# bitsauce/Carla-ppo

Measured on AMD Instinct MI355X. Metric: VAE+PPO train frames/sec on 160×80×3 synthetic obs at 1/2/4/8 MI355X, higher is better.
Workload: dtype bf16; 1 GPU; ConvVAE SGD step (fwd+ELBO+bwd+TF-Adam), batch=512 per GPU, 160x80x3 frames, z_dim=64, rgb target (BASELINE configs[1]; global batch 512); global_batch=512, parallelism=single, frames_resident_in_hbm=2048, frame_table=uint8 camera bytes, k/255 in registers, noise=N(0,1) drawn inside the reparameterisation kernel (Philox4x32-10), launch=eager launches: one C call per step (mi_vae_train_step), storage=bf16 activations/weights, fp32 accumulate, fp32 master weights+Adam

## Files before the change

### carla-ppo_amd/csrc/conv_ops.hip

```cpp
#include <stdlib.h>
#include "gemm_core.hpp"
#include "tallk_tile.hpp"
#include "mi_internal.hpp"
#include "mi355_carla.h"

using namespace mi;

namespace {

inline int esz_of(int dtype) { return dtype == MI_BF16 ? 2 : 4; }
inline bool dtype_ok(int dtype) { return dtype == MI_F32 || dtype == MI_BF16 || dtype == MI_BF16X3; }

template <typename T, typename TIn, int AMODE, int BMODE, int VA, int AALIGN>
int launch_gemm_bn(hipStream_t st, const GemmParams& p, int M_for_grid, int gz) {
    const int gx = (M_for_grid + GEMM_BM - 1) / GEMM_BM;
    if (gx <= 0) return MI_OK;
    if (p.N <= 32) {
        dim3 g(gx, 1, gz);
        MI_LAUNCH((gemm_kernel<T, TIn, AMODE, BMODE, VA, AALIGN, 32>), g, dim3(GEMM_NT), 0, st, p);
    } else if (p.N <= 64) {
        dim3 g(gx, 1, gz);
        MI_LAUNCH((gemm_kernel<T, TIn, AMODE, BMODE, VA, AALIGN, 64>), g, dim3(GEMM_NT), 0, st, p);
    } else {
        dim3 g(gx, (p.N + 127) / 128, gz);
// ... 141 lines not shown
    if (j == 0) { f.first[0] = 0; f.ovw = 0; }
    if (overwrite) f.ovw |= 1u << j;
    f.slabs[j] = slabs; f.out[j] = out; f.stride[j] = stride; f.n[j] = n; f.nslab[j] = nslab;
    f.kl[j] = sr_kl(n, nslab);
    f.vec[j] = ((((uintptr_t)slabs) | ((uintptr_t)out)) & 15) == 0 && stride % 4 == 0;
    const long long quads = (n + 3) / 4;
    f.first[j + 1] = f.first[j] + (int)((quads * f.kl[j] + 255) / 256);
}
struct PendingReduce { TapWgradParams q; int splits, ngroups, kind; const float* bpart; float* bout; int bnslab, bN; };
struct PendingFold { const float* tmp; float* out; const float* tmp_bias; float* dbias; int T, R, Q, NB; };
static thread_local PendingFold g_folds[16];
static thread_local int g_nfolds = 0;
__global__ __launch_bounds__(256) void fold_split_kernel(const PendingFold f) {
    const long long n = (long long)f.T * f.R * f.Q;
    const long long i = (long long)blockIdx.x * 256 + threadIdx.x;
    if (i < n) {
        const int q = (int)(i % f.Q); const long long tr = i / f.Q; const int r = (int)(tr % f.R); const long long t = tr / f.R;
        const float* s = f.tmp + ((t * 2 * f.R + 2 * r) * 2ll * f.Q + 2 * q);
        f.out[i] += (s[0] + s[1]) + (s[2ll * f.Q] + s[2ll * f.Q + 1]);
    } else if (f.dbias && i - n < f.NB) {
        const int b = (int)(i - n);
        f.dbias[b] += f.tmp_bias[2 * b] + f.tmp_bias[2 * b + 1];
    }
}
static int launch_fold(hipStream_t st, const PendingFold& f) {
    const long long n = (long long)f.T * f.R * f.Q + (f.dbias ? f.NB : 0);
    MI_LAUNCH(fold_split_kernel, dim3((unsigned)((n + 255) / 256)), dim3(256), 0, st, f);
    return mi_check_launch("fold_split_kernel");
}
static thread_local PendingReduce g_pending[16];
static thread_local int g_npending = 0, g_defer_reduces = 0, g_defer_pause = 0;
static unsigned reduce_ry(const PendingReduce& r) {
    unsigned ry = 1;
    while (((unsigned)(r.ngroups / 512 + 1) * ry < 512 || r.splits / (int)ry > 16) && (int)(ry * 2) <= r.splits / 4 && ry < (unsigned)knob(K_REDUCE_RY_CAP)) ry *= 2;
    return ry;
}
static unsigned reduce_blocks(const PendingReduce& r, unsigned ry) { const unsigned upb = 256 / ry, nunits = (unsigned)r.ngroups / 2; return (nunits + upb - 1) / upb; }
static void launch_tiled_reduce(hipStream_t st, const PendingReduce& r) {
    const unsigned ry = reduce_ry(r);
    const dim3 rg(reduce_blocks(r, ry), 1, 1);
    if (r.kind == 0) MI_LAUNCH((reduce_tiled_kernel<TC_CONV, 2, 4, 2>), rg, dim3(256), 0, st, r.q, r.splits, r.ngroups, (int)ry);
    else if (r.kind == 1) MI_LAUNCH((reduce_tiled_kernel<TC_GATHER, 2, 4, 2>), rg, dim3(256), 0, st, r.q, r.splits, r.ngroups, (int)ry);
    else MI_LAUNCH((reduce_tiled_kernel<TC_GATHER, 3, 2, 4>), rg, dim3(256), 0, st, r.q, r.splits, r.ngroups, (int)ry);
    if (r.bpart) mi_reduce_slabs(st, r.bpart, (long long)r.bN, r.bnslab, (long long)r.bN, r.bout);
}
extern "C" int mi_tapwgrad_defer(int on) {
    const int prev = g_defer_reduces;
    g_defer_reduces = on ? 1 : 0;
    g_npending = 0; g_nfolds = 0; g_defer_pause = 0;
    return prev;
}
extern "C" int mi_tapwgrad_defer_pause(int pause) { const int prev = g_defer_pause; g_defer_pause = pause ? 1 : 0; return prev; }
static thread_local int t_slab_bf16 = -1;
static inline int slab_bf16_now() { return t_slab_bf16 >= 0 ? t_slab_bf16 : knob(K_SLAB_BF16_DEFAULT); }
extern "C" int mi_tapwgrad_slab_bf16(int on) { const int prev = t_slab_bf16; t_slab_bf16 = on < 0 ? -1 : (on ? 1 : 0); return prev; }
static int tapwgrad_flush_reduces(void* stream);
extern "C" int mi_tapwgrad_flush(void* stream) {
    int rc = tapwgrad_flush_reduces(stream);
    const int nf = g_nfolds;
    g_nfolds = 0;
    for (int i = 0; i < nf && rc == MI_OK; ++i) rc = launch_fold((hipStream_t)stream, g_folds[i]);
    return rc;
}
static int tapwgrad_flush_reduces(void* stream) {
    const int n = g_npending;
    g_npending = 0;
    if (n == 0) return MI_OK;
    if (n == 1 || n > TW_MAX_FUSED) {
        for (int i = 0; i < n; ++i) launch_tiled_reduce((hipStream_t)stream, g_pending[i]);
        return mi_check_launch("reduce_tiled_kernel");
    }
    static thread_local FusedReduceParams f;
    f.n = n; f.first[0] = 0; f.bias.njobs = 0; f.bias.first[0] = 0; f.bias.ovw = 0;
    for (int i = 0; i < n; ++i) {
        const PendingReduce& r = g_pending[i];
        f.q[i] = r.q; f.splits[i] = r.splits; f.ngroups[i] = r.ngroups; f.kind[i] = r.kind; f.ry[i] = (int)reduce_ry(r);
        f.first[i + 1] = f.first[i] + (int)reduce_blocks(r, (unsigned)f.ry[i]);
        if (r.bpart && f.bias.njobs < SR_MAX) sr_add(f.bias, r.bpart, (long long)r.bN, r.bnslab, (long long)r.bN, r.bout);
    }
    for (int i = n; i < TW_MAX_FUSED; ++i) f.first[i + 1] = f.first[n];
    for (int i = f.bias.njobs; i < SR_MAX; ++i) f.bias.first[i + 1] = f.bias.first[f.bias.njobs];
    MI_LAUNCH(reduce_fused_kernel, dim3((unsigned)(f.first[n] + f.bias.first[f.bias.njobs])), dim3(256), 0, (hipStream_t)stream, f);
    return mi_check_launch("reduce_fused_kernel");
}

int try_tapwgrad(hipStream_t st, int dtype, int mode, const void* a, const void* d, int B, int IH, int IW, int C, int OH, int OW, int N,
                 int KH, int KW, float* out, void* scratch, long long scratch_bytes, float* dbias) {
    if (!knob(K_TAPWGRAD) || dtype != MI_BF16) return 0;
    if (KH != KW || KH < 3 || KH > 6) return 0;
    if ((((uintptr_t)a) & 15) || (((uintptr_t)d) & 15) || C % 8 != 0 || N % 8 != 0) return 0;
    TapWgradParams q = {};
    const int taps = (KH + 1) / 2;
    int KCB, NEB;
    if (mode == TC_CONV) {
        if (taps != 2 || (4 * C) % 128 != 0 || N % 64 != 0) return 0;
        q.GH = OH + 1; q.GW = OW + 1; q.HY = q.HX = 0; q.KC = 4 * C; q.NE = N; KCB = 128; NEB = 64;
    } else {
        q.HY = q.HX = taps - 1;
        q.GH = (OH + 1) / 2 + q.HY; q.GW = (OW + 1) / 2 + q.HX; q.KC = C; q.NE = 4 * N;
        if (taps == 2) { if (C % 128 != 0 || N % 64 != 0) return 0; KCB = 128; NEB = 64; }
        else { if (C % 64 != 0 || N != 32) return 0; KCB = 64; NEB = 128; }
    }
    if ((taps - 1) * q.GW + taps - 1 > TC_MAXHALO) return 0;
    const long long MP = (long long)B * q.GH * q.GW, a_bytes = (long long)B * IH * IW * C * 2, d_bytes = (long long)B * OH * OW * N * 2;
    if (MP >= (1ll << 30) || !fits_desc(a_bytes) || !fits_desc(d_bytes)) return 0;
    q.a = a; q.a_bytes = (uint32_t)a_bytes; q.d = d; q.d_bytes = (uint32_t)d_bytes;
    q.B = B; q.IH = IH; q.IW = IW; q.C = C; q.OH = OH; q.OW = OW; q.N = N; q.KH = KH; q.KW = KW; q.MP = (int)MP;
    q.nkb = q.KC / KCB;
    const int gy = q.nkb * (q.NE / NEB);
    const int ntb = NEB / 32;
    q.npairs = 0;
    for (int tap = 0; tap < taps * taps; ++tap)
        for (int nt = 0; nt < ntb; ++nt) {
            bool valid = true;
            if (mode == TC_GATHER && NEB == 4 * N) {
                const int ta = tap / taps, tb = tap % taps;
                valid = (nt >> 1) + 2 * (q.HY - ta) < KH && (nt & 1) + 2 * (q.HX - tb) < KW;
            }
            if (valid) {
                if (q.npairs >= 32) return 0;
                bool first = true;
                for (int k = 0; k < q.npairs; ++k) if (q.pair_nt[k] == nt) first = false;
                q.pair_tap[q.npairs] = (unsigned char)tap; q.pair_nt[q.npairs] = (unsigned char)nt; q.pair_first[q.npairs] = first ? 1 : 0; ++q.npairs;
            }
        }
    {
        unsigned char t2[32], n2[32], f2[32];
        int k = 0;
        for (int pass = 0; pass < 2; ++pass)
            for (int i = 0; i < q.npairs; ++i)
                if ((q.pair_first[i] != 0) == (pass == 0)) { t2[k] = q.pair_tap[i]; n2[k] = q.pair_nt[i]; f2[k] = q.pair_first[i]; ++k; }
        for (int i = 0; i < q.npairs; ++i) { q.pair_tap[i] = t2[i]; q.pair_nt[i] = n2[i]; q.pair_first[i] = f2[i]; }
    }
    q.dbias = dbias;
    int splits = knob(K_TAPWGRAD_BLOCKS) / gy; if (splits < 1) splits = 1;
    long long pps = (MP + splits - 1) / splits; pps = (pps + TW_BP - 1) / TW_BP * TW_BP;
    splits = (int)((MP + pps - 1) / pps);
    q.pos_per_split = (int)pps;
    q.div_g = make_fastdiv(q.GH); q.div_gw = make_fastdiv(q.GW); q.div_n = make_fastdiv(N);
    q.div_2c = make_fastdiv(2 * C); q.div_c = make_fastdiv(C);
    q.out = out;
    q.trace = g_trace; q.trace_cap = g_trace_cap; q.dbg_cheap_addr = (knob(K_WGRAD_DBG) >= 2 && knob(K_WGRAD_DBG) <= 5) ? knob(K_WGRAD_DBG) : 0;
    const int kt_tiles = taps == 2 ? 4 : 2;
    const long long slab_floats = (long long)gy * q.npairs * kt_tiles * 1024;
    q.slabs = nullptr; q.slab_stride = slab_floats; q.slab_bf16 = slab_bf16_now() ? 1 : 0;
    const bool split = knob(K_TAPWGRAD_SPLIT) && taps == 2 && q.npairs == 8;
    const long long slab_bytes = ((long long)splits * slab_floats * (q.slab_bf16 ? 2 : 4) + 255) / 256 * 256;
    q.bias_part = nullptr; q.bias_nh = split ? 2 : 1;
    const long long bias_bytes = dbias ? (long long)splits * q.bias_nh * q.NE * 4 : 0;
    if (scratch && splits > 1 && (((uintptr_t)scratch) & 15) == 0 && scratch_bytes >= slab_bytes + bias_bytes && slab_floats < (1ll << 29) && (!dbias || N <= 256)) {
        q.slabs = (float*)scratch;
        if (dbias) q.bias_part = (float*)((char*)scratch + slab_bytes);
    }
    q.gx = splits; q.gy = gy;
    dim3 g((unsigned)((splits + 7) / 8 * 8 * gy), 1, 1);
    const bool ldec = (knob(K_TW_LDEC) & 1) && !q.dbg_cheap_addr && !q.trace, ldec_cw = (knob(K_TW_LDEC) & 2) && !q.dbg_cheap_addr && !q.trace;
    const bool dbg = q.dbg_cheap_addr != 0;
    if (mode == TC_CONV) {
        if (split && dbg) MI_LAUNCH((tapwgrad_kernel<TC_CONV, 2, 4, 2, 2, true, false, true>), g, dim3(TW_NT), 0, st, q);
        else if (split && ldec) MI_LAUNCH((tapwgrad_kernel<TC_CONV, 2, 4, 2, 2, true, true>), g, dim3(TW_NT), 0, st, q);
        else if (split) MI_LAUNCH((tapwgrad_kernel<TC_CONV, 2, 4, 2, 2, true>), g, dim3(TW_NT), 0, st, q);
        else MI_LAUNCH((tapwgrad_kernel<TC_CONV, 2, 4, 2, 1>), g, dim3(TW_NT), 0, st, q);
    } else if (taps == 2) {
        if (split && dbg) MI_LAUNCH((tapwgrad_kernel<TC_GATHER, 2, 4, 2, 2, true, false, true>), g, dim3(TW_NT), 0, st, q);
        else if (split && ldec) MI_LAUNCH((tapwgrad_kernel<TC_GATHER, 2, 4, 2, 2, true, true>), g, dim3(TW_NT), 0, st, q);
        else if (split) MI_LAUNCH((tapwgrad_kernel<TC_GATHER, 2, 4, 2, 2, true>), g, dim3(TW_NT), 0, st, q);
        else MI_LAUNCH((tapwgrad_kernel<TC_GATHER, 2, 4, 2, 1>), g, dim3(TW_NT), 0, st, q);
    }
    else {
        if (q.npairs > 32) return 0;
        if (knob(K_TAPWGRAD_CW) && KH == 5 && C == 64 && q.NE == 128 && q.KC == 64 && q.slabs) {
            if (dbg) MI_LAUNCH((tapwgrad_cw_kernel<false, true>), g, dim3(TWC_NT), 0, st, q);
            else if (ldec_cw) MI_LAUNCH(tapwgrad_cw_kernel<true>, g, dim3(TWC_NT), 0, st, q); else MI_LAUNCH(tapwgrad_cw_kernel<false>, g, dim3(TWC_NT), 0, st, q);
        }
        else MI_LAUNCH((tapwgrad_kernel<TC_GATHER, 3, 2, 4, 4>), g, dim3(TW_NT), 0, st, q);
    }
    int rc = mi_check_launch("tapwgrad_kernel");
    if (rc == MI_OK && q.slabs) {
        PendingReduce r;
        r.q = q; r.splits = splits; r.ngroups = (int)(slab_floats / 4); r.kind = mode == TC_CONV ? 0 : (taps == 2 ? 1 : 2);
        r.bpart = q.bias_part; r.bout = dbias; r.bnslab = splits * q.bias_nh * (q.NE / N); r.bN = N;
        if (g_defer_reduces && !g_defer_pause && g_npending < 16) g_pending[g_npending++] = r;
        else { launch_tiled_reduce(st, r); rc = mi_check_launch("reduce_tiled_kernel"); }
    }
    return rc == MI_OK ? 1 : rc;
}

int try_tapwgrad_split(hipStream_t st, int mode, const void* a, const void* d, int B, int IH, int IW, int C, int OH, int OW, int N,
                       int KH, int KW, float* out, void* scratch, long long scratch_bytes, float* dbias) {
    const int on = knob(K_X3_TAPWGRAD);
    if (!on || !scratch || (((uintptr_t)scratch) & 255)) return 0;
    const long long nw = (long long)KH * KW * C * N;
    const long long tmp_bytes = ((4 * nw + 2 * N) * 4 + 255) / 256 * 256;
    if (scratch_bytes < tmp_bytes + (1 << 20)) return 0;
    const int taps = (KH + 1) / 2;
    if (KH != KW || taps != 2) return 0;
    if (mode == TC_CONV ? ((8 * C) % 128 != 0 || (2 * N) % 64 != 0) : ((2 * C) % 128 != 0 || (2 * N) % 64 != 0)) return 0;
    if (on != 2 && (mode != TC_CONV || (long long)C * N > 64 * 128)) return 0;
    float* tmp = (float*)scratch; float* tb = tmp + 4 * nw;
    if (hipMemsetAsync(tmp, 0, (size_t)((4 * nw + 2 * N) * 4), st) != hipSuccess) return mi_fail(MI_ERR_LAUNCH, "try_tapwgrad_split: memset failed");
    const int r = try_tapwgrad(st, MI_BF16, mode, a, d, B, IH, IW, 2 * C, OH, OW, 2 * N, KH, KW, tmp, (char*)scratch + tmp_bytes, scratch_bytes - tmp_bytes, dbias ? tb : nullptr);
    if (r <= 0) return r;
    PendingFold f = {tmp, out, tb, dbias, KH * KW, mode == TC_CONV ? C : N, mode == TC_CONV ? N : C, N};
    if (g_defer_reduces && !g_defer_pause && g_nfolds < 16) { g_folds[g_nfolds++] = f; return 1; }
    const int rc = launch_fold(st, f);
    return rc == MI_OK ? 1 : rc;
}

template <typename T, int TAPS, int CPR>
int launch_gather_narrow(hipStream_t st, const TapParams& q) {
    dim3 g((q.MP + GN_BMT - 1) / GN_BMT);
    if (q.N == 3 && sizeof(T) == 2 && q.labels && q.loss_kind == 0 && knob(K_NARROW_LEAN)) MI_LAUNCH((gather_narrow_kernel<T, TAPS, CPR, 3, true>), g, dim3(GN_NT), 0, st, q);
    else if (q.N == 3) MI_LAUNCH((gather_narrow_kernel<T, TAPS, CPR, 3>), g, dim3(GN_NT), 0, st, q);
    else if (q.N == 1) MI_LAUNCH((gather_narrow_kernel<T, TAPS, CPR, 1>), g, dim3(GN_NT), 0, st, q);
    else MI_LAUNCH((gather_narrow_kernel<T, TAPS, CPR, 0>), g, dim3(GN_NT), 0, st, q);
    return mi_check_launch("gather_narrow_kernel");
}

struct NarrowLoss {
    const float* labels; const int* idx; long long stride; int kind; float inv_b; void* dlogits; float* lpart; float* bpart; int cap; int nblocks;
// ... 790 lines not shown
```

### carla-ppo_amd/csrc/mi_internal.hpp

```cpp
#pragma once
#include <hip/hip_runtime.h>
#include <hip/hip_ext.h>
#include "tuning.hpp"

enum { MI_F32 = 0, MI_BF16 = 1, MI_BF16X3 = 2 };
enum { MI_OK = 0, MI_ERR_ARG = -1, MI_ERR_SHAPE = -2, MI_ERR_LAUNCH = -3, MI_ERR_STATE = -4 };

extern thread_local hipEvent_t mi_tl_stop_event;
#define MI_LAUNCH(kernel, grid, block, shmem, stream, ...) do { \
        if (mi_tl_stop_event) { const hipEvent_t ev__ = mi_tl_stop_event; mi_tl_stop_event = nullptr; \
            hipExtLaunchKernelGGL(kernel, grid, block, shmem, stream, nullptr, ev__, 0, __VA_ARGS__); } \
        else hipLaunchKernelGGL(kernel, grid, block, shmem, stream, __VA_ARGS__); } while (0)

const void* mi_rwconv_take_wfrag();
bool mi_enc12_eligible(int dtype, int B, int FH, int FW);
int mi_fail(int code, const char* msg);
int mi_check_launch(const char* what);

extern "C" int mi_tapwgrad_defer(int on);
extern "C" int mi_tapwgrad_flush(void* stream);
extern "C" int mi_tapwgrad_defer_pause(int pause);
extern "C" int mi_tapwgrad_slab_bf16(int on);

int mi_try_rwconv_gather(hipStream_t st, int dtype, const void* a, const void* w, int B, int IH, int IW, int C, int OH, int OW, int N,
                         int KH, int KW, void* out, const float* bias, const void* mask, int relu, const void* mask_bits, void* bits_out, const void* wfrag);
int mi_try_rwconv_conv(hipStream_t st, int dtype, const void* a, const void* w, int B, int IH, int IW, int C, int OH, int OW, int N,
                       int KH, int KW, int ldb, void* out, const float* bias, const void* mask, int relu, const void* wfrag);
void mi_get_trace(long long** buf, int* cap);

int mi_reduce_slabs(hipStream_t st, const float* slabs, long long stride, int nslab, long long n, float* out, int overwrite = 0);
extern "C" int mi_small_reduce_defer(int on);
extern "C" int mi_small_reduce_flush(void* stream);
extern "C" int mi_small_reduce_bind(void* stream);
extern "C" int mi_small_reduce_deferring(void);
```

### carla-ppo_amd/csrc/tapwgrad_tile.hpp

```cpp
#pragma once
#include <type_traits>
#include "tapconv_tile.hpp"
#include "wgrad_tile.hpp"

namespace mi {

constexpr int TW_BP = 128;
constexpr int TW_NT = 512;
constexpr int TW_MAXPAIR = 32;

struct TapWgradParams {
    const void* a; uint32_t a_bytes;
    const void* d; uint32_t d_bytes;
    int B, IH, IW, C;
    int OH, OW, N;
    int KH, KW;
    int GH, GW, HY, HX;
    int KC, NE, MP;
    int nkb;
    int gx, gy;
    int pos_per_split;
    int npairs;
    unsigned char pair_tap[TW_MAXPAIR], pair_nt[TW_MAXPAIR], pair_first[TW_MAXPAIR];
    float* dbias;
    FastDiv div_g, div_gw, div_n, div_2c, div_c;
    float* out;
    float* slabs; long long slab_stride;
    float* bias_part; int bias_nh;
    int slab_bf16;
    long long* trace; int trace_cap;
    int dbg_cheap_addr;
};

#ifdef MI355_TW_SLAB_PLAIN
#define TW_SLAB_STORE(v, ptr) (*(ptr) = (v))
#else
#define TW_SLAB_STORE(v, ptr) __builtin_nontemporal_store((v), (ptr))
#endif
typedef uint32_t u32x4 __attribute__((ext_vector_type(4)));
typedef uint32_t tw_u32x2 __attribute__((ext_vector_type(2)));
__device__ __forceinline__ u32x4 make_srd(const void* base, uint32_t bytes) {
    const unsigned long long b = (unsigned long long)base;
    u32x4 r;
    r[0] = (uint32_t)b; r[1] = (uint32_t)(b >> 32) & 0xffffu; r[2] = bytes; r[3] = 0x00020000u;
    r[0] = __builtin_amdgcn_readfirstlane(r[0]); r[1] = __builtin_amdgcn_readfirstlane(r[1]);
    r[2] = __builtin_amdgcn_readfirstlane(r[2]); r[3] = __builtin_amdgcn_readfirstlane(r[3]);
    return r;
}
__device__ __forceinline__ void dma16_asm(const u32x4 srd, uint32_t lds_addr, uint32_t voff) {
    asm volatile("s_mov_b32 m0, %0\n\ts_nop 0\n\tbuffer_load_dwordx4 %1, %2, 0 offen lds"
                 :: "s"(lds_addr), "v"(voff), "s"(srd) : "memory", "m0");
}

template <int CPR> __device__ __forceinline__ int tw_swz(int row) {
    return CPR == 16 ? (row & 3) << 2 : ((row >> 1) & 1) << 2;
}

template <int MODE, int TAPS>
__device__ __forceinline__ bool tw_dw_index(const TapWgradParams& p, int kc0, int ne0, int tap, int kt, int nt, int row, int lcol, long long& base, long long& stride) {
    const int ta = tap / TAPS, tb = tap % TAPS;
    if constexpr (MODE == TC_CONV) {
        const int kc = kc0 + kt * 32 + row, ne = ne0 + nt * 32 + lcol;
        uint32_t phh, rem, pww, c;
        p.div_2c.divmod((uint32_t)(kc < p.KC ? kc : 0), phh, rem);
        p.div_c.divmod(rem, pww, c);
        const int kh = 2 * ta + (int)phh, kw = 2 * tb + (int)pww;
        base = ((long long)(kh * p.KW + kw) * p.C + c) * p.N + ne; stride = p.N;
        return kc < p.KC && ne < p.NE && kh < p.KH && kw < p.KW;
    } else {
        const int ne = ne0 + nt * 32 + row, kc = kc0 + kt * 32 + lcol;
        uint32_t cls, n;
        p.div_n.divmod((uint32_t)(ne < p.NE ? ne : 0), cls, n);
        const int kh = (int)(cls >> 1) + 2 * (p.HY - ta), kw = (int)(cls & 1) + 2 * (p.HX - tb);
        base = ((long long)(kh * p.KW + kw) * p.N + n) * p.C + kc; stride = p.C;
        return kc < p.KC && ne < p.NE && kh < p.KH && kw < p.KW;
    }
}

template <int MODE, int TAPS, int KT, int NTB, int PPW, bool SPLIT = false, bool LDEC = false, bool DBG = false>
__global__ __launch_bounds__(TW_NT) void tapwgrad_kernel(const TapWgradParams p) {
    const int dbgm = DBG ? p.dbg_cheap_addr : 0;
    static_assert(!SPLIT || (TAPS == 2 && NTB == 2 && PPW == NTB), "split layout: 4 taps x 2 position halves = 8 waves");
    typedef bf16_t T;
    constexpr int ESZ = 2, VE = 8;
    constexpr int KCB = 32 * KT, NEB = 32 * NTB;
    constexpr int PA = KCB * ESZ, PD = NEB * ESZ;
    constexpr int CPA = PA / 16, CPD = PD / 16;
    constexpr int SPI_A = 1024 / PA, SPI_D = 1024 / PD;
    constexpr int MAXSLOT = TW_BP + TC_MAXHALO;
    constexpr int NIA = (MAXSLOT / SPI_A + 7) / 8;
    constexpr int NID = TW_BP / SPI_D / 8;
    constexpr int ASTAGE = MAXSLOT * PA, DSTAGE = TW_BP * PD, STAGE = ASTAGE + DSTAGE;
    static_assert(NID >= 1 && 2 * STAGE <= 160 * 1024, "tile config");

    __shared__ __attribute__((aligned(1024))) unsigned char lds[2 * STAGE];

    const int tid = threadIdx.x, lane = tid & 63;
    const int wave = __builtin_amdgcn_readfirstlane(tid >> 6);
    int tr_n = 0;
    const int bslot = (int)blockIdx.x >> 3;
    const int by = bslot % p.gy, bx = (bslot / p.gy) * 8 + ((int)blockIdx.x & 7);
    if (bx >= p.gx) return;
    long long* const tr = p.trace ? p.trace + ((long long)(by * p.gx + bx) * 8 + (tid >> 6)) * 32 : nullptr;
    const bool tr_on = tr && ((long long)(by * p.gx + bx) * 8 + 8) * 32 <= p.trace_cap && lane == 0;
#define TW_STAMP() do { if (tr_on && tr_n < 32) tr[tr_n++] = (long long)__builtin_amdgcn_s_memtime(); } while (0)
    TW_STAMP();
#ifdef MI355_TW_EPI_STAMPS
#define TW_EPI_STAMP() TW_STAMP()
#else
#define TW_EPI_STAMP() do {} while (0)
#endif
    const int kb = by % p.nkb, nb = by / p.nkb;
    const int kc0 = kb * KCB, ne0 = nb * NEB;
    const int Pbeg = bx * p.pos_per_split;
    const int Pend = min(p.MP, Pbeg + p.pos_per_split);
    if (Pbeg >= Pend) return;
    const int nsteps = (Pend - Pbeg + TW_BP - 1) / TW_BP;
    const int halo = (TAPS - 1) * p.GW + TAPS - 1;
    const int ninstrA = (TW_BP + halo + SPI_A - 1) / SPI_A;

    const u32x4 rsA = make_srd(p.a, p.a_bytes), rsD = make_srd(p.d, p.d_bytes);
    const uint32_t lds0 = (uint32_t)(uintptr_t)(__attribute__((address_space(3))) unsigned char*)lds;

    const int rA = lane / CPA, cA = (lane % CPA) ^ tw_swz<CPA>(rA);
    const int rD = lane / CPD, cD = (lane % CPD) ^ tw_swz<CPD>(rD);
    uint32_t a_koff; int a_sub = 0; bool a_kok;
    {
        const int kc = kc0 + cA * VE;
        a_kok = kc < p.KC;
        if constexpr (MODE == TC_CONV) {
            uint32_t phh, r, pww, c;
            p.div_2c.divmod((uint32_t)(a_kok ? kc : 0), phh, r);
            p.div_c.divmod(r, pww, c);
            a_koff = (phh * p.IW * p.C + r) * ESZ; a_sub = (int)(phh * 2 + pww);
        } else a_koff = (uint32_t)kc * ESZ;
    }
    uint32_t d_koff; int d_cls = 0; bool d_kok;
    {
        const int ne = ne0 + cD * VE;
        d_kok = ne < p.NE;
        if constexpr (MODE == TC_CONV) d_koff = (uint32_t)ne * ESZ;
        else {
            uint32_t cls, n;
            p.div_n.divmod((uint32_t)(d_kok ? ne : 0), cls, n);
            d_cls = (int)cls;
            d_koff = ((((cls >> 1) * p.OW + (cls & 1)) * p.N) + n) * ESZ;
        }
    }
    auto issue_one = [&](int step, int buf, int idx) {
        const int Ps = Pbeg + step * TW_BP;
        const uint32_t As = lds0 + buf * STAGE, Ds = As + ASTAGE;
        if (dbgm == 3) return;
        if (dbgm == 2) {
            const int t = wave + 8 * (idx < NIA ? idx : idx - NIA);
            if (idx < NIA && t >= ninstrA) return;
            const uint32_t vo = (uint32_t)((Ps * 64 + t * 1024 + lane * 16) & 0xFFFFF);
            if (idx < NIA) dma16_asm(rsA, As + t * 1024, vo); else dma16_asm(rsD, Ds + t * 1024, vo);
            return;
        }
        if (idx < NIA) {
            const int t = wave + 8 * idx;
            if (t >= ninstrA) return;
            const int P = Ps + SPI_A * t + rA;
            const bool ok = P < p.MP && a_kok;
            uint32_t g, gx, b, gy;
            p.div_gw.divmod((uint32_t)(ok ? P : 0), g, gx);
            p.div_g.divmod(g, b, gy);
            uint32_t vo;
            if constexpr (MODE == TC_CONV) {
                const int y = 2 * (int)gy + (a_sub >> 1), x = 2 * (int)gx + (a_sub & 1);
                const bool v = ok && y < p.IH && x < p.IW;
                vo = v ? (((b * p.IH + 2 * gy) * p.IW + 2 * gx) * p.C) * ESZ + a_koff : G2_OOB;
            } else {
                const int iy = (int)gy - p.HY, ix = (int)gx - p.HX;
                const bool v = ok && iy >= 0 && iy < p.IH && ix >= 0 && ix < p.IW;
                vo = v ? (((b * p.IH + iy) * p.IW + ix) * p.C) * ESZ + a_koff : G2_OOB;
            }
            dma16_asm(rsA, As + t * 1024, vo);
        } else {
            const int t = wave + 8 * (idx - NIA);
            const int P = Ps + SPI_D * t + rD;
            const bool ok = P < Pend && d_kok;
            uint32_t g, gx, b, gy;
            p.div_gw.divmod((uint32_t)(ok ? P : 0), g, gx);
            p.div_g.divmod(g, b, gy);
            uint32_t vo;
            if constexpr (MODE == TC_CONV) {
                const bool v = ok && (int)gy < p.OH && (int)gx < p.OW;
                vo = v ? (((b * p.OH + gy) * p.OW + gx) * p.N) * ESZ + d_koff : G2_OOB;
            } else {
                const int oy = 2 * (int)gy + (d_cls >> 1), ox = 2 * (int)gx + (d_cls & 1);
                const bool v = ok && oy < p.OH && ox < p.OW;
                vo = v ? (((b * p.OH + 2 * gy) * p.OW + 2 * gx) * p.N) * ESZ + d_koff : G2_OOB;
            }
            dma16_asm(rsD, Ds + t * 1024, vo);
        }
    };
    constexpr int NDMA = NIA + NID, NKS = SPLIT ? TW_BP / 32 : TW_BP / 16;
    constexpr int RA = NIA * SPI_A, RD = NID * SPI_D;
    static_assert(!LDEC || RA + RD <= 64, "lane-parallel row decode: one lane per requested row");
    const bool lpA = lane < RA;
    const int lpj = lpA ? lane : lane - RA;
    const int lpt = wave + 8 * (lpA ? lpj / SPI_A : lpj / SPI_D);
    const int lprow = lpA ? SPI_A * lpt + lpj % SPI_A : SPI_D * lpt + lpj % SPI_D;
    const bool lplive = lane < RA + RD && (!lpA || lpt < ninstrA);
    auto decode_rows = [&](int step) -> uint32_t {
        const int P = Pbeg + step * TW_BP + lprow;
        const bool ok = lplive && P < (lpA ? p.MP : Pend);
        uint32_t g, gx, b, gy;
        p.div_gw.divmod((uint32_t)(ok ? P : 0), g, gx);
        p.div_g.divmod(g, b, gy);
        if constexpr (MODE == TC_CONV) {
            const int yy = lpA ? 2 * (int)gy : (int)gy, xx = lpA ? 2 * (int)gx : (int)gx;
            const int H = lpA ? p.IH : p.OH, W = lpA ? p.IW : p.OW, CB = (lpA ? p.C : p.N) * ESZ;
            const bool v = ok && yy < H && xx < W;
            const uint32_t edge = lpA ? (uint32_t)(yy + 1 >= H) | ((uint32_t)(xx + 1 >= W) << 1) : 0u;
            return v ? (uint32_t)(((int)b * H + yy) * W + xx) * (uint32_t)CB | edge : G2_OOB;
        } else {
            const int yy = lpA ? (int)gy - p.HY : 2 * (int)gy, xx = lpA ? (int)gx - p.HX : 2 * (int)gx;
            const int H = lpA ? p.IH : p.OH, W = lpA ? p.IW : p.OW, CB = (lpA ? p.C : p.N) * ESZ;
            const bool v = ok && yy >= 0 && yy < H && xx >= 0 && xx < W;
            const uint32_t edge = lpA ? 0u : (uint32_t)(yy + 1 >= H) | ((uint32_t)(xx + 1 >= W) << 1);
            return v ? (uint32_t)(((int)b * H + yy) * W + xx) * (uint32_t)CB | edge : G2_OOB;
        }
    };
    const uint32_t a_edge = MODE == TC_CONV ? (uint32_t)((a_sub >> 1) | ((a_sub & 1) << 1)) : 0u;
    const uint32_t d_edge = MODE == TC_CONV ? 0u : (uint32_t)((d_cls >> 1) | ((d_cls & 1) << 1));
    uint32_t lp_offs = 0;
    auto fetch_row = [&](int idx) -> uint32_t {
        const int src = idx < NIA ? idx * SPI_A + rA : RA + (idx - NIA) * SPI_D + rD;
        return (uint32_t)__builtin_amdgcn_ds_bpermute(src * 4, (int)lp_offs);
    };
    auto issue_row = [&](int buf, int idx, uint32_t row) {
        const uint32_t As = lds0 + buf * STAGE, Ds = As + ASTAGE;
        if (idx < NIA) {
            const int t = wave + 8 * idx;
            if (t >= ninstrA) return;
            const bool bad = (row & a_edge) != 0u || !a_kok;
            dma16_asm(rsA, As + t * 1024, bad ? G2_OOB : (row & ~3u) + a_koff);
        } else {
            const int t = wave + 8 * (idx - NIA);
            const bool bad = (row & d_edge) != 0u || !d_kok;
            dma16_asm(rsD, Ds + t * 1024, bad ? G2_OOB : (row & ~3u) + d_koff);
        }
    };
    uint32_t lp_nn = 0;

    const int trow0 = (lane >> 5) * 8 + ((lane & 15) >> 2);
    const int tcol = ((lane >> 4) & 1) * 16 + (lane & 3) * 4;
    int pr_tap[PPW], pr_nt[PPW];
    bool pr_on[PPW], pr_bias[PPW];
    uint32_t aoff[PPW][KT], doff[PPW];
    const int half = SPLIT ? (wave & 1) : 0;
    const int trow = trow0 + 64 * half;
#pragma unroll
    for (int q = 0; q < PPW; ++q) {
        if constexpr (SPLIT) {
            pr_on[q] = true; pr_tap[q] = wave >> 1; pr_nt[q] = q;
            pr_bias[q] = q == 0 && p.dbias && kb == 0 && (wave >> 1) < 2;
        } else {
            const int pi = wave + 8 * q;
            pr_on[q] = pi < p.npairs;
            pr_tap[q] = pr_on[q] ? p.pair_tap[pi] : 0;
            pr_nt[q] = pr_on[q] ? p.pair_nt[pi] : 0;
            pr_bias[q] = pr_on[q] && p.dbias && kb == 0 && p.pair_first[pi];
        }
        const int ta = pr_tap[q] / TAPS, tb = pr_tap[q] % TAPS;
        const int row = trow + ta * p.GW + tb;
#pragma unroll
        for (int kt = 0; kt < KT; ++kt) {
            const int col = kt * 32 + tcol;
            aoff[q][kt] = (uint32_t)(row * PA + ((((col >> 3) ^ tw_swz<CPA>(row))) << 4) + (col & 7) * ESZ);
        }
        const int col = pr_nt[q] * 32 + tcol;
        doff[q] = (uint32_t)(ASTAGE + trow * PD + ((((col >> 3) ^ tw_swz<CPD>(trow))) << 4) + (col & 7) * ESZ);
    }

    f32x16 acc[PPW][KT];
#pragma unroll
    for (int q = 0; q < PPW; ++q)
#pragma unroll
        for (int kt = 0; kt < KT; ++kt)
#pragma unroll
            for (int r = 0; r < 16; ++r) acc[q][kt][r] = 0.f;

    constexpr int NBQ = 1;
    const int bias_nt = SPLIT ? (wave >> 1) & 1 : 0;
    f32x16 accb[NBQ];
#pragma unroll
    for (int q = 0; q < NBQ; ++q)
#pragma unroll
        for (int r = 0; r < 16; ++r) accb[q][r] = 0.f;
    bool any_bias = false;
#pragma unroll
    for (int q = 0; q < NBQ; ++q) any_bias = any_bias || pr_bias[q];
    const u16x8 ones = {0x3F80, 0x3F80, 0x3F80, 0x3F80, 0x3F80, 0x3F80, 0x3F80, 0x3F80};

    typedef __attribute__((address_space(3))) s16x4* lds_v4;
    if constexpr (LDEC) {
        lp_offs = decode_rows(0);
#pragma unroll
        for (int i = 0; i < NDMA; ++i) issue_row(0, i, fetch_row(i));
        lp_offs = decode_rows(1);
    } else {
#pragma unroll
        for (int i = 0; i < NDMA; ++i) issue_one(0, 0, i);
    }
    TW_STAMP();
    constexpr int ND = SPLIT ? PPW : 1;
    constexpr int NU = SPLIT ? NKS : NKS * PPW;
    constexpr int NKI = NKS;
    constexpr bool PIPE = true;
    struct Frag { u16x8 d[ND]; u16x8 a[KT]; };
    auto tr_read = [&](uint32_t off, int pitch) -> u16x8 {
        const s16x4 lo = __builtin_amdgcn_ds_read_tr16_b64_v4i16((lds_v4)(lds + off));
        const s16x4 hi = __builtin_amdgcn_ds_read_tr16_b64_v4i16((lds_v4)(lds + off + 4 * pitch));
        u16x8 f;
#pragma unroll
        for (int e = 0; e < 4; ++e) { f[e] = (unsigned short)lo[e]; f[4 + e] = (unsigned short)hi[e]; }
        return f;
    };
    auto load_unit = [&](Frag& f, uint32_t sbase, int u) {
        const int ks = SPLIT ? u : u / PPW, q = SPLIT ? 0 : u % PPW;
#pragma unroll
        for (int j = 0; j < ND; ++j) f.d[j] = tr_read(sbase + doff[SPLIT ? j : q] + ks * 16 * PD, PD);
#pragma unroll
        for (int kt = 0; kt < KT; ++kt) f.a[kt] = tr_read(sbase + aoff[q][kt] + ks * 16 * PA, PA);
    };
    auto run_steps = [&](auto bias_c) {
        constexpr bool BIAS = decltype(bias_c)::value;
        for (int step = 0; step < nsteps; ++step) {
            const int cur = step & 1;
            asm volatile("s_waitcnt vmcnt(0)" ::: "memory");
            __syncthreads();
            if (step < 4) TW_STAMP();
            const bool more = step + 1 < nsteps;
            const uint32_t sbase = (uint32_t)(cur * STAGE);
            Frag fr[2];
            if constexpr (PIPE) load_unit(fr[0], sbase, 0);
            if constexpr (LDEC) {
                lp_nn = decode_rows(step + 2);
                asm volatile("" : "+v"(lp_nn));
            }
#pragma unroll
            for (int u = 0; u < NU; ++u) {
                const int ks = SPLIT ? u : u / PPW, q0 = SPLIT ? 0 : u % PPW;
                if constexpr (LDEC) {
                    if (more && (SPLIT || q0 == 0) && ks < NKI) {
                        uint32_t rows[(NDMA + NKI - 1) / NKI];
#pragma unroll
                        for (int i = ks, g = 0; i < NDMA; i += NKI, ++g) rows[g] = fetch_row(i);
#pragma unroll
                        for (int i = ks, g = 0; i < NDMA; i += NKI, ++g) issue_row(cur ^ 1, i, rows[g]);
                    }
                } else
                if (more && (SPLIT || q0 == 0) && ks < NKI) {
#pragma unroll
                    for (int i = ks; i < NDMA; i += NKI) issue_one(step + 1, cur ^ 1, i);
                }
                if (dbgm == 4) continue;
                if constexpr (!PIPE) load_unit(fr[u & 1], sbase, u);
                else if (u + 1 < NU) load_unit(fr[(u + 1) & 1], sbase, u + 1);
                const Frag& f = fr[u & 1];
#pragma unroll
                for (int j = 0; j < ND; ++j) {
                    const int q = SPLIT ? j : q0;
                    if constexpr (BIAS) {
                        if (q == 0) {
                            u16x8 dsel = f.d[j];
                            if constexpr (SPLIT) dsel = bias_nt ? f.d[1] : f.d[0];
                            accb[0] = __builtin_amdgcn_mfma_f32_32x32x16_bf16(__builtin_bit_cast(bf16x8, ones), __builtin_bit_cast(bf16x8, dsel), accb[0], 0, 0, 0);
                        }
                    }
#pragma unroll
                    for (int kt = 0; kt < KT; ++kt) {
                        if constexpr (MODE == TC_CONV)
                            acc[q][kt] = __builtin_amdgcn_mfma_f32_32x32x16_bf16(__builtin_bit_cast(bf16x8, f.a[kt]), __builtin_bit_cast(bf16x8, f.d[j]), acc[q][kt], 0, 0, 0);
                        else
                            acc[q][kt] = __builtin_amdgcn_mfma_f32_32x32x16_bf16(__builtin_bit_cast(bf16x8, f.d[j]), __builtin_bit_cast(bf16x8, f.a[kt]), acc[q][kt], 0, 0, 0);
                    }
                }
                if constexpr (LDEC) {
                    if (u == NU - 1) lp_offs = lp_nn;
                }
            }
        }
    };
    if (any_bias) run_steps(std::true_type{}); else run_steps(std::false_type{});
    TW_STAMP();
    const int lcol = lane & 31, lgrp = lane >> 5;
#pragma unroll
    for (int q = 0; q < NBQ; ++q) {
        if (!pr_bias[q] || lane >= 32) continue;
        const int ne = ne0 + (SPLIT ? bias_nt : pr_nt[q]) * 32 + lane;
        if (ne >= p.NE) continue;
        int n = ne;
        if constexpr (MODE == TC_GATHER) n = ne - (int)p.div_n.div((uint32_t)ne) * p.N;
        if (p.bias_part) p.bias_part[((long long)bx * p.bias_nh + (SPLIT ? half : 0)) * p.NE + ne] = accb[q][0];
        else atomicAdd(&p.dbias[n], accb[q][0]);
    }
    auto emit = [&](const f32x16 (&tiles)[KT], int tap, int nt, int pi) {
        if (dbgm == 5) return;
        if (p.slabs) {
            const long long eoff = (long long)bx * p.slab_stride + ((long long)(by * p.npairs + pi) * KT) * 1024 + lane * 4;
            if (p.slab_bf16) {
                bf16_t* const dst = (bf16_t*)p.slabs + eoff;
#pragma unroll
                for (int kt = 0; kt < KT; ++kt)
#pragma unroll
                    for (int g4 = 0; g4 < 4; ++g4) {
                        const float v[4] = {tiles[kt][4 * g4], tiles[kt][4 * g4 + 1], tiles[kt][4 * g4 + 2], tiles[kt][4 * g4 + 3]};
                        TW_SLAB_STORE(__builtin_bit_cast(tw_u32x2, pack4<bf16_t>(v)), (tw_u32x2*)(dst + (kt * 4 + g4) * 256));
                    }
                return;
            }
            float* const dst = p.slabs + eoff;
#pragma unroll
            for (int kt = 0; kt < KT; ++kt)
#pragma unroll
                for (int g4 = 0; g4 < 4; ++g4) {
                    const f32x4 v = {tiles[kt][4 * g4], tiles[kt][4 * g4 + 1], tiles[kt][4 * g4 + 2], tiles[kt][4 * g4 + 3]};
                    __builtin_nontemporal_store(v, (f32x4*)(dst + (kt * 4 + g4) * 256));
                }
            return;
        }
#pragma unroll
        for (int kt = 0; kt < KT; ++kt) {
#pragma unroll
            for (int g4 = 0; g4 < 4; ++g4) {
                long long base, stride;
                const bool ok = tw_dw_index<MODE, TAPS>(p, kc0, ne0, tap, kt, nt, 8 * g4 + 4 * lgrp, lcol, base, stride);
#pragma unroll
                for (int t = 0; t < 4; ++t)
                    if (ok) atomicAdd(p.out + base + t * stride, tiles[kt][4 * g4 + t]);
            }
        }
    };
    if constexpr (SPLIT) {
        constexpr int WSZ = KT * 16 * 64;
        static_assert(8 * WSZ * 4 <= 2 * STAGE, "reduction scratch");
        __syncthreads();
        TW_EPI_STAMP();
        float* const red = (float*)lds;
#pragma unroll
        for (int kt = 0; kt < KT; ++kt)
#pragma unroll
            for (int r = 0; r < 16; ++r) red[wave * WSZ + (kt * 16 + r) * 64 + lane] = half ? acc[0][kt][r] : acc[1][kt][r];
        TW_EPI_STAMP();
        __syncthreads();
        TW_EPI_STAMP();
        f32x16 fin[KT];
#pragma unroll
        for (int kt = 0; kt < KT; ++kt)
#pragma unroll
            for (int r = 0; r < 16; ++r) fin[kt][r] = (half ? acc[1][kt][r] : acc[0][kt][r]) + red[(wave ^ 1) * WSZ + (kt * 16 + r) * 64 + lane];
        TW_EPI_STAMP();
        emit(fin, wave >> 1, half, (wave >> 1) * 2 + half);
    } else {
#pragma unroll
        for (int q = 0; q < PPW; ++q) {
            if (!pr_on[q]) continue;
            emit(acc[q], pr_tap[q], pr_nt[q], wave + 8 * q);
        }
    }
    TW_STAMP();
#undef TW_STAMP
#undef TW_EPI_STAMP
// ... 405 lines not shown
```

Before: 686,500 frames/s.

## Iterate tap-wgrad over dense output positions instead of padded slot grid

The tap-based weight-gradient kernel now splits work over the dense output positions (MQ = B*DH*DW) rather than the padded slot grid (MP). This avoids spending MFMA steps on halo and padding slots. Each step maps its dense range back to slot rows for the A-tile loads, sized by a precomputed nrows span. Per-lane A fragment row offsets are decoded each step and shared across lanes with ds_bpermute, so the static aoff table is gone. A host-side plan function computes splits and row spans, and the 5x5 channel-wise shape keeps the old split logic. The cost is extra divmod work, bpermute traffic and register pressure per step.

```diff
diff --git a/carla-ppo_amd/csrc/conv_ops.hip b/carla-ppo_amd/csrc/conv_ops.hip
--- a/carla-ppo_amd/csrc/conv_ops.hip
+++ b/carla-ppo_amd/csrc/conv_ops.hip
@@ -247,6 +247,33 @@
     for (int i = f.bias.njobs; i < SR_MAX; ++i) f.bias.first[i + 1] = f.bias.first[f.bias.njobs];
     MI_LAUNCH(reduce_fused_kernel, dim3((unsigned)(f.first[n] + f.bias.first[f.bias.njobs])), dim3(256), 0, (hipStream_t)stream, f);
     return mi_check_launch("reduce_fused_kernel");
+}
+
+struct TapWgradPlan { int GH, GW, DH, DW, halo, nrows, splits, steps; long long MP, MQ, pos_per_split; };
+static TapWgradPlan tapwgrad_plan(int mode, int taps, int B, int OH, int OW, int gy, int target_blocks) {
+    TapWgradPlan pl = {};
+    if (mode == TC_CONV) { pl.GH = OH + 1; pl.GW = OW + 1; pl.DH = OH; pl.DW = OW; }
+    else { pl.DH = (OH + 1) / 2; pl.DW = (OW + 1) / 2; pl.GH = pl.DH + taps - 1; pl.GW = pl.DW + taps - 1; }
+    pl.halo = (taps - 1) * pl.GW + taps - 1;
+    pl.MP = (long long)B * pl.GH * pl.GW; pl.MQ = (long long)B * pl.DH * pl.DW;
+    const long long F = (long long)pl.DH * pl.DW;
+    const long long span = (TW_BP - 1) + (long long)((TW_BP - 1 + pl.DW - 1) / pl.DW) * (pl.GW - pl.DW) + ((TW_BP - 1 + F - 1) / F) * (long long)(pl.GH - pl.DH) * pl.GW;
+    const long long nrows = span + pl.halo + 1;
+    pl.nrows = nrows > (1 << 20) ? (1 << 20) : (int)nrows;
+    int splits = target_blocks / (gy > 0 ? gy : 1); if (splits < 1) splits = 1;
+    long long pps = (pl.MQ + splits - 1) / splits; pps = (pps + TW_BP - 1) / TW_BP * TW_BP; if (pps < TW_BP) pps = TW_BP;
+    pl.splits = (int)((pl.MQ + pps - 1) / pps); pl.pos_per_split = pps; pl.steps = (int)(pps / TW_BP);
+    return pl;
+}
+extern "C" int mi_tapwgrad_plan(int mode, int B, int OH, int OW, int C, int N, int KH, int target_blocks, int* out) {
+    const int taps = (KH + 1) / 2;
+    if (!out || B < 1 || OH < 1 || OW < 1 || taps != 2 || KH < 3 || (mode != TC_CONV && mode != TC_GATHER)) return 0;
+    if (C % 8 != 0 || N % 64 != 0 || (mode == TC_CONV ? (4 * C) % 128 != 0 : C % 128 != 0)) return 0;
+    const int gy = mode == TC_CONV ? (4 * C / 128) * (N / 64) : (C / 128) * (4 * N / 64);
+    const TapWgradPlan pl = tapwgrad_plan(mode, taps, B, OH, OW, gy, target_blocks > 0 ? target_blocks : knob(K_TAPWGRAD_BLOCKS));
+    if (pl.halo > TC_MAXHALO || pl.nrows > TW_BP + TC_MAXHALO || pl.MP >= (1ll << 30)) return 0;
+    out[0] = pl.DH; out[1] = pl.DW; out[2] = (int)pl.MQ; out[3] = pl.splits; out[4] = (int)pl.pos_per_split; out[5] = pl.steps; out[6] = pl.nrows; out[7] = gy;
+    return 1;
 }
 
 int try_tapwgrad(hipStream_t st, int dtype, int mode, const void* a, const void* d, int B, int IH, int IW, int C, int OH, int OW, int N,
@@ -298,9 +325,20 @@
         for (int i = 0; i < q.npairs; ++i) { q.pair_tap[i] = t2[i]; q.pair_nt[i] = n2[i]; q.pair_first[i] = f2[i]; }
     }
     q.dbias = dbias;
-    int splits = knob(K_TAPWGRAD_BLOCKS) / gy; if (splits < 1) splits = 1;
-    long long pps = (MP + splits - 1) / splits; pps = (pps + TW_BP - 1) / TW_BP * TW_BP;
-    splits = (int)((MP + pps - 1) / pps);
+    const TapWgradPlan pl = tapwgrad_plan(mode, taps, B, OH, OW, gy, knob(K_TAPWGRAD_BLOCKS));
+    if (pl.GH != q.GH || pl.GW != q.GW) return mi_fail(MI_ERR_LAUNCH, "try_tapwgrad: plan and launcher disagree on the slot grid");
+    const bool cw_shape = mode == TC_GATHER && taps == 3 && knob(K_TAPWGRAD_CW) && KH == 5 && C == 64 && q.NE == 128 && q.KC == 64;
+    int splits; long long pps;
+    if (cw_shape) {
+        splits = knob(K_TAPWGRAD_BLOCKS) / gy; if (splits < 1) splits = 1;
+        pps = (MP + splits - 1) / splits; pps = (pps + TW_BP - 1) / TW_BP * TW_BP;
+        splits = (int)((MP + pps - 1) / pps);
+    } else {
+        if (pl.nrows > TW_BP + TC_MAXHALO) return 0;
+        splits = pl.splits; pps = pl.pos_per_split;
+    }
+    q.DH = pl.DH; q.DW = pl.DW; q.MQ = (int)pl.MQ; q.nrows = pl.nrows;
+    q.div_dh = make_fastdiv(pl.DH); q.div_dw = make_fastdiv(pl.DW);
     q.pos_per_split = (int)pps;
     q.div_g = make_fastdiv(q.GH); q.div_gw = make_fastdiv(q.GW); q.div_n = make_fastdiv(N);
     q.div_2c = make_fastdiv(2 * C); q.div_c = make_fastdiv(C);
diff --git a/carla-ppo_amd/csrc/mi_internal.hpp b/carla-ppo_amd/csrc/mi_internal.hpp
--- a/carla-ppo_amd/csrc/mi_internal.hpp
+++ b/carla-ppo_amd/csrc/mi_internal.hpp
@@ -21,6 +21,7 @@
 extern "C" int mi_tapwgrad_flush(void* stream);
 extern "C" int mi_tapwgrad_defer_pause(int pause);
 extern "C" int mi_tapwgrad_slab_bf16(int on);
+extern "C" int mi_tapwgrad_plan(int mode, int B, int OH, int OW, int C, int N, int KH, int target_blocks, int* out);
 
 int mi_try_rwconv_gather(hipStream_t st, int dtype, const void* a, const void* w, int B, int IH, int IW, int C, int OH, int OW, int N,
                          int KH, int KW, void* out, const float* bias, const void* mask, int relu, const void* mask_bits, void* bits_out, const void* wfrag);
diff --git a/carla-ppo_amd/csrc/tapwgrad_tile.hpp b/carla-ppo_amd/csrc/tapwgrad_tile.hpp
--- a/carla-ppo_amd/csrc/tapwgrad_tile.hpp
+++ b/carla-ppo_amd/csrc/tapwgrad_tile.hpp
@@ -17,13 +17,15 @@
     int KH, KW;
     int GH, GW, HY, HX;
     int KC, NE, MP;
+    int DH, DW, MQ;
+    int nrows;
     int nkb;
     int gx, gy;
     int pos_per_split;
     int npairs;
     unsigned char pair_tap[TW_MAXPAIR], pair_nt[TW_MAXPAIR], pair_first[TW_MAXPAIR];
     float* dbias;
-    FastDiv div_g, div_gw, div_n, div_2c, div_c;
+    FastDiv div_g, div_gw, div_n, div_2c, div_c, div_dh, div_dw;
     float* out;
     float* slabs; long long slab_stride;
     float* bias_part; int bias_nh;
@@ -113,11 +115,17 @@
     const int kb = by % p.nkb, nb = by / p.nkb;
     const int kc0 = kb * KCB, ne0 = nb * NEB;
     const int Pbeg = bx * p.pos_per_split;
-    const int Pend = min(p.MP, Pbeg + p.pos_per_split);
+    const int Pend = min(p.MQ, Pbeg + p.pos_per_split);
     if (Pbeg >= Pend) return;
     const int nsteps = (Pend - Pbeg + TW_BP - 1) / TW_BP;
-    const int halo = (TAPS - 1) * p.GW + TAPS - 1;
-    const int ninstrA = (TW_BP + halo + SPI_A - 1) / SPI_A;
+    const int ninstrA = (p.nrows + SPI_A - 1) / SPI_A;
+    auto slot_of = [&](uint32_t q) -> int {
+        uint32_t R, gx, b, gy;
+        p.div_dw.divmod(q, R, gx);
+        p.div_dh.divmod(R, b, gy);
+        return (int)((b * (uint32_t)p.GH + gy) * (uint32_t)p.GW + gx);
+    };
+    int S0n = __builtin_amdgcn_readfirstlane(slot_of((uint32_t)Pbeg));
 
     const u32x4 rsA = make_srd(p.a, p.a_bytes), rsD = make_srd(p.d, p.d_bytes);
     const uint32_t lds0 = (uint32_t)(uintptr_t)(__attribute__((address_space(3))) unsigned char*)lds;
@@ -161,7 +169,7 @@
         if (idx < NIA) {
             const int t = wave + 8 * idx;
             if (t >= ninstrA) return;
-            const int P = Ps + SPI_A * t + rA;
+            const int P = S0n + SPI_A * t + rA;
             const bool ok = P < p.MP && a_kok;
             uint32_t g, gx, b, gy;
             p.div_gw.divmod((uint32_t)(ok ? P : 0), g, gx);
@@ -181,14 +189,13 @@
             const int t = wave + 8 * (idx - NIA);
             const int P = Ps + SPI_D * t + rD;
             const bool ok = P < Pend && d_kok;
-            uint32_t g, gx, b, gy;
-            p.div_gw.divmod((uint32_t)(ok ? P : 0), g, gx);
-            p.div_g.divmod(g, b, gy);
             uint32_t vo;
             if constexpr (MODE == TC_CONV) {
-                const bool v = ok && (int)gy < p.OH && (int)gx < p.OW;
-                vo = v ? (((b * p.OH + gy) * p.OW + gx) * p.N) * ESZ + d_koff : G2_OOB;
+                vo = ok ? (uint32_t)P * (uint32_t)(p.N * ESZ) + d_koff : G2_OOB;
             } else {
+                uint32_t g, gx, b, gy;
+                p.div_dw.divmod((uint32_t)(ok ? P : 0), g, gx);
+                p.div_dh.divmod(g, b, gy);
                 const int oy = 2 * (int)gy + (d_cls >> 1), ox = 2 * (int)gx + (d_cls & 1);
                 const bool v = ok && oy < p.OH && ox < p.OW;
                 vo = v ? (((b * p.OH + 2 * gy) * p.OW + 2 * gx) * p.N) * ESZ + d_koff : G2_OOB;
@@ -205,11 +212,13 @@
     const int lprow = lpA ? SPI_A * lpt + lpj % SPI_A : SPI_D * lpt + lpj % SPI_D;
     const bool lplive = lane < RA + RD && (!lpA || lpt < ninstrA);
     auto decode_rows = [&](int step) -> uint32_t {
-        const int P = Pbeg + step * TW_BP + lprow;
+        const int q0 = Pbeg + step * TW_BP;
+        const int P = (lpA ? slot_of((uint32_t)q0) : q0) + lprow;
         const bool ok = lplive && P < (lpA ? p.MP : Pend);
+        const FastDiv dvw = lpA ? p.div_gw : p.div_dw, dvh = lpA ? p.div_g : p.div_dh;
         uint32_t g, gx, b, gy;
-        p.div_gw.divmod((uint32_t)(ok ? P : 0), g, gx);
-        p.div_g.divmod(g, b, gy);
+        dvw.divmod((uint32_t)(ok ? P : 0), g, gx);
+        dvh.divmod(g, b, gy);
         if constexpr (MODE == TC_CONV) {
             const int yy = lpA ? 2 * (int)gy : (int)gy, xx = lpA ? 2 * (int)gx : (int)gx;
             const int H = lpA ? p.IH : p.OH, W = lpA ? p.IW : p.OW, CB = (lpA ? p.C : p.N) * ESZ;
@@ -250,7 +259,7 @@
     const int tcol = ((lane >> 4) & 1) * 16 + (lane & 3) * 4;
     int pr_tap[PPW], pr_nt[PPW];
     bool pr_on[PPW], pr_bias[PPW];
-    uint32_t aoff[PPW][KT], doff[PPW];
+    uint32_t doff[PPW];
     const int half = SPLIT ? (wave & 1) : 0;
     const int trow = trow0 + 64 * half;
 #pragma unroll
@@ -265,13 +274,6 @@
             pr_nt[q] = pr_on[q] ? p.pair_nt[pi] : 0;
             pr_bias[q] = pr_on[q] && p.dbias && kb == 0 && p.pair_first[pi];
         }
-        const int ta = pr_tap[q] / TAPS, tb = pr_tap[q] % TAPS;
-        const int row = trow + ta * p.GW + tb;
-#pragma unroll
-        for (int kt = 0; kt < KT; ++kt) {
-            const int col = kt * 32 + tcol;
-            aoff[q][kt] = (uint32_t)(row * PA + ((((col >> 3) ^ tw_swz<CPA>(row))) << 4) + (col & 7) * ESZ);
-        }
         const int col = pr_nt[q] * 32 + tcol;
         doff[q] = (uint32_t)(ASTAGE + trow * PD + ((((col >> 3) ^ tw_swz<CPD>(trow))) << 4) + (col & 7) * ESZ);
     }
@@ -320,12 +322,63 @@
         for (int e = 0; e < 4; ++e) { f[e] = (unsigned short)lo[e]; f[4 + e] = (unsigned short)hi[e]; }
         return f;
     };
+    constexpr int NTQ = SPLIT ? 1 : PPW;
+    constexpr int NRG = SPLIT ? 1 : 2;
+    constexpr int NER = 2 * NKS;
+    constexpr bool EAHEAD = NTQ * NER <= 16;
+    static_assert(STAGE % 1024 == 0, "row offsets carry the stage base: its low bits must be clear for the XOR");
+    int eshift[NTQ];
+#pragma unroll
+    for (int t = 0; t < NTQ; ++t) eshift[t] = (pr_tap[t] / TAPS) * p.GW + pr_tap[t] % TAPS;
+    uint32_t ekt[KT];
+#pragma unroll
+    for (int kt = 0; kt < KT; ++kt) { const int col = kt * 32 + tcol; ekt[kt] = (uint32_t)(((col >> 3) << 4) + (col & 7) * ESZ); }
+    uint32_t edec[NTQ][NRG], erow[NTQ][NER], erown[EAHEAD ? NTQ : 1][EAHEAD ? NER : 1];
+    auto decode_erows = [&](int step) {
+        const int q0 = Pbeg + step * TW_BP;
+        const int s0 = slot_of((uint32_t)q0);
+#pragma unroll
+        for (int g = 0; g < NRG; ++g) {
+            const int rel = slot_of((uint32_t)(q0 + 64 * (SPLIT ? half : g) + lane)) - s0;
+#pragma unroll
+            for (int t = 0; t < NTQ; ++t) {
+                const int row = rel + eshift[t];
+                edec[t][g] = (uint32_t)((step & 1) * STAGE + row * PA + (tw_swz<CPA>(row) << 4));
+            }
+        }
+    };
+    auto collect_erows = [&](uint32_t (&dst)[EAHEAD ? NTQ : 1][EAHEAD ? NER : 1], uint32_t (&cur)[NTQ][NER]) {
+#pragma unroll
+        for (int t = 0; t < NTQ; ++t)
+#pragma unroll
+            for (int e = 0; e < NER; ++e) {
+                const int ks = e >> 1, src = trow0 + 16 * (ks & 3) + 4 * (e & 1);
+                const uint32_t v = (uint32_t)__builtin_amdgcn_ds_bpermute(src * 4, (int)edec[t][SPLIT ? 0 : ks >> 2]);
+                if constexpr (EAHEAD) dst[t][e] = v; else cur[t][e] = v;
+            }
+    };
+    decode_erows(0);
+    if constexpr (EAHEAD) {
+        collect_erows(erown, erow);
+#pragma unroll
+        for (int t = 0; t < NTQ; ++t)
+#pragma unroll
+            for (int e = 0; e < NER; ++e) erow[t][e] = erown[t][e];
+    }
+    auto tr_read2 = [&](uint32_t lo_off, uint32_t hi_off) -> u16x8 {
+        const s16x4 lo = __builtin_amdgcn_ds_read_tr16_b64_v4i16((lds_v4)(lds + lo_off));
+        const s16x4 hi = __builtin_amdgcn_ds_read_tr16_b64_v4i16((lds_v4)(lds + hi_off));
+        u16x8 f;
+#pragma unroll
+        for (int e = 0; e < 4; ++e) { f[e] = (unsigned short)lo[e]; f[4 + e] = (unsigned short)hi[e]; }
+        return f;
+    };
     auto load_unit = [&](Frag& f, uint32_t sbase, int u) {
         const int ks = SPLIT ? u : u / PPW, q = SPLIT ? 0 : u % PPW;
 #pragma unroll
         for (int j = 0; j < ND; ++j) f.d[j] = tr_read(sbase + doff[SPLIT ? j : q] + ks * 16 * PD, PD);
 #pragma unroll
-        for (int kt = 0; kt < KT; ++kt) f.a[kt] = tr_read(sbase + aoff[q][kt] + ks * 16 * PA, PA);
+        for (int kt = 0; kt < KT; ++kt) f.a[kt] = tr_read2(erow[q][2 * ks] ^ ekt[kt], erow[q][2 * ks + 1] ^ ekt[kt]);
     };
     auto run_steps = [&](auto bias_c) {
         constexpr bool BIAS = decltype(bias_c)::value;
@@ -337,7 +390,11 @@
             const bool more = step + 1 < nsteps;
             const uint32_t sbase = (uint32_t)(cur * STAGE);
             Frag fr[2];
+            if constexpr (!EAHEAD) collect_erows(erown, erow);
             if constexpr (PIPE) load_unit(fr[0], sbase, 0);
+            S0n = __builtin_amdgcn_readfirstlane(slot_of((uint32_t)(Pbeg + (step + 1) * TW_BP)));
+            decode_erows(step + 1);
+            if constexpr (EAHEAD) collect_erows(erown, erow);
             if constexpr (LDEC) {
                 lp_nn = decode_rows(step + 2);
                 asm volatile("" : "+v"(lp_nn));
@@ -383,6 +440,12 @@
                 if constexpr (LDEC) {
                     if (u == NU - 1) lp_offs = lp_nn;
                 }
+            }
+            if constexpr (EAHEAD) {
+#pragma unroll
+                for (int t = 0; t < NTQ; ++t)
+#pragma unroll
+                    for (int e = 0; e < NER; ++e) erow[t][e] = erown[t][e];
             }
         }
     };
```

Result: slower. 650,200 frames/s (-5.3%).
